# salemon/quattro-transformer-ilqr

Measured on AMD Instinct MI355X. Metric: iLQR iterations/sec (batch x horizon steps/s), quadrotor N=50 batch=4096, higher is better.
Workload: dtype f32; 1 GPU; quadrotor n_x=12 n_u=4 N=50, pure iLQR iteration = simulate (nominal rollout + cost) + linearisation and Riccati sweep (one fused launch) + 6-alpha line search/commit (BASELINE configs[2]; configs[3] when n_gpus=8); batch_per_gpu=4096, global_batch=4096, horizon=50, n_x=12, n_u=4, integrator=euler, parallelism=dp1 (independent trajectory shards)

## Files before the change

### quattro-transformer-ilqr_amd/csrc/quattro_device.h

```cpp
#pragma once
#include <hip/hip_runtime.h>

#include "../../include/quattro_hip.h"

#define QT_WAVE 64

#define QT_HD __host__ __device__ __forceinline__

template <int NX, int NU>
struct RowMajorRec {
  static constexpr int NZ = NX + NU;
  static constexpr int A = 0;
  static constexpr int B = A + NX * NX;
  static constexpr int LXX = B + NX * NU;
  static constexpr int LUX = LXX + NX * NX;
  static constexpr int LUU = LUX + NU * NX;
  static constexpr int LX = LUU + NU * NU;
  static constexpr int LU = LX + NX;
  static constexpr int SIZE = LU + NU;
  static constexpr int STRIDE = (SIZE + 3) / 4 * 4;
  static QT_HD int a(int i, int j) { return A + i * NX + j; }
  static QT_HD int b(int i, int a_) { return B + i * NU + a_; }
  static QT_HD int lxx(int i, int j) { return LXX + i * NX + j; }
  static QT_HD int lux(int a_, int j) { return LUX + a_ * NX + j; }
  static QT_HD int luu(int a_, int b_) { return LUU + a_ * NU + b_; }
  static QT_HD int lx(int i) { return LX + i; }
  static QT_HD int lu(int a_) { return LU + a_; }
};

struct Tile16Rec {
  static constexpr int NX = 12, NU = 4;
  static constexpr int F = 0, LXB = 192, LUU = 384, LZ = 400, SIZE = 416, STRIDE = 416;
  static QT_HD int zcol(int z) { return z < 12 ? (z / 3) * 4 + z % 3 : 4 * (z - 12) + 3; }
  static QT_HD int f(int i, int z) { return F + 3 * (16 * (i / 3) + zcol(z)) + i % 3; }
  static QT_HD int a(int i, int j) { return f(i, j); }
  static QT_HD int b(int i, int a_) { return f(i, 12 + a_); }
  static QT_HD int lxx(int i, int j) { return LXB + 4 * (12 * (i / 3) + j) + i % 3; }
  static QT_HD int lux(int a_, int j) { return LXB + 4 * (12 * a_ + j) + 3; }
  static QT_HD int luu(int a_, int b_) { return LUU + 4 * a_ + b_; }
  static QT_HD int lx(int i) { return LZ + i; }
  static QT_HD int lu(int a_) { return LZ + 12 + a_; }
};

struct Tile16CRec {
  static constexpr int NX = 12, NU = 4;
  static constexpr int F = 0, NDYN = 14, DUMP = 43, LUU = 44, LZ = 60, SIZE = 76, STRIDE = 76;
  static constexpr int HEADER = Tile16Rec::STRIDE;
  static QT_HD int dyn_index(int lane) {
    switch (lane) {
      case 19: return 0;  case 23: return 1;  case 24: return 2;  case 25: return 3;  case 26: return 4;
      case 27: return 5;  case 31: return 6;  case 40: return 7;  case 41: return 8;  case 45: return 9;
      case 46: return 10; case 60: return 11; case 61: return 12; case 62: return 13;
      default: return -1;
    }
// ... 51 lines not shown
struct PlantSpec {
  int integrator;
  float phys[8];
};

struct RefRows {
  const float* rows;
  int R, s, preview;
};
__device__ __forceinline__ int qt_ref_row(const RefRows& rr, int t) {
  const int i = rr.s + rr.preview * t;
  return i < rr.R - 1 ? i : rr.R - 1;
}
struct NoRef {
  __device__ __forceinline__ void operator()(int) const {}
};

namespace {
struct AlphaList {
  float a[QUATTRO_MAX_ALPHAS];
};
inline AlphaList make_alpha_list(const float* alphas, int n_alpha) {
  AlphaList al;
  for (int i = 0; i < QUATTRO_MAX_ALPHAS; ++i) al.a[i] = i < n_alpha ? alphas[i] : 0.0f;
  return al;
}
}

#define QT_DISPATCH_INTEG(p, ...)                                 \
  if ((p).integrator == QUATTRO_INTEGRATOR_EULER) {               \
    constexpr bool RK4 = false;                                   \
    __VA_ARGS__;                                                  \
  } else if ((p).integrator == QUATTRO_INTEGRATOR_RK4) {          \
    constexpr bool RK4 = true;                                    \
    __VA_ARGS__;                                                  \
  } else {                                                        \
    return QUATTRO_ERR_UNSUPPORTED;                               \
  }

__device__ __forceinline__ float qt_readlane(float v, int lane) {
  return __int_as_float(__builtin_amdgcn_readlane(__float_as_int(v), lane));
}

__device__ __forceinline__ float qt_sum_rows(float v) {
  int vi = __float_as_int(v);
  auto s16 = __builtin_amdgcn_permlane16_swap(vi, vi, false, false);
  float a = __int_as_float(s16[0]) + __int_as_float(s16[1]);
  int ai = __float_as_int(a);
  auto s32 = __builtin_amdgcn_permlane32_swap(ai, ai, false, false);
  return __int_as_float(s32[0]) + __int_as_float(s32[1]);
}

__device__ __forceinline__ bool qt_finite(float v) { return fabsf(v) <= 3.0e38f; }
```

### quattro-transformer-ilqr_amd/csrc/rollout_quad.hip

```cpp
#include "rollout_quad_body.h"

namespace {

template <bool RK4>
__global__ __launch_bounds__(64) void simulate_quad_kernel(const quattro_model_params p, const float* __restrict__ x0,
                                                           const float* __restrict__ u, int B, int N,
                                                           float* __restrict__ x, double* __restrict__ cost) {
  const int gid = blockIdx.x * blockDim.x + threadIdx.x;
  simulate_quad_body<RK4>(p, x0, u, N, x, cost, gid, (gid >> 2) < B);
}

template <bool RK4>
__global__ __launch_bounds__(64) void rollout_quad_kernel(const quattro_model_params p, const float* __restrict__ x_nom,
                                                          const float* __restrict__ u_nom, const float* __restrict__ K,
                                                          const float* __restrict__ k, AlphaList al, int n_alpha, int B,
                                                          int N, float* __restrict__ x_new, float* __restrict__ u_new,
                                                          double* __restrict__ cost, const int32_t* __restrict__ active) {
  const int gid = blockIdx.x * blockDim.x + threadIdx.x;
  const int b = gid >> 5, ai = (gid >> 2) & 7;
  const bool live = (b < B) && (active == nullptr || active[b < B ? b : 0] != 0);
  if (!__any(live)) return;
  const bool mine = live && ai < n_alpha;
  const size_t bb = live ? b : 0;
  const int aa = mine ? ai : 0;
  const LaneConst L = lane_const(p, gid & 3);
  const float* xn = x_nom + bb * (N + 1) * NX;
  const float* un = u_nom + bb * N * NU;
  const int wb = __builtin_amdgcn_readfirstlane(b);
  const NomSrc nom(L, x_nom, u_nom, K, k, N, wb, live ? b - wb : 0, 2);
  float alpha = al.a[0];
#pragma unroll
  for (int i = 1; i < QUATTRO_MAX_ALPHAS; ++i) alpha = (aa == i) ? al.a[i] : alpha;
  double J;
  if (x_new != nullptr && u_new != nullptr) {
    float* xo = x_new + ((size_t)aa * B + bb) * (N + 1) * NX;
    float* uo = u_new + ((size_t)aa * B + bb) * N * NU;
    if (mine && L.j < 3) {
#pragma unroll
      for (int g = 0; g < 4; ++g) xo[3 * g + L.a] = xn[3 * g + L.a];
    }
    J = quad_rollout_closed<RK4, 4, true, RK4>(p, L, nom, alpha, N, mine, ArrayStore(L, xo, uo, mine));
  } else {
    J = quad_rollout_closed<RK4, 4, true, RK4>(p, L, nom, alpha, N, mine, NoStore{});
  }
  J = quad_sum(J);
  if (mine && L.j == 0) cost[(size_t)ai * B + b] = J;
}

template <bool RK4>
__global__ __launch_bounds__(64) void linesearch_quad_kernel(const quattro_model_params p, float* x_nom, float* u_nom,
                                                             const float* __restrict__ K, const float* __restrict__ k,
                                                             AlphaList al, int n_alpha, int B, int N, double tol,
                                                             double* cost, int32_t* __restrict__ alpha_idx,
                                                             int32_t* active, int32_t* iters,
                                                             float* __restrict__ scratch) {
  linesearch_quad_body<RK4, 4, true, false, false, RK4>(p, x_nom, u_nom, K, k, al, n_alpha, B, N, tol, cost, alpha_idx, active, iters, scratch,
                                     blockIdx.x * blockDim.x + threadIdx.x, false);
}

__global__ __launch_bounds__(64) void track_quad_kernel(const float dt, const PlantSpec plant, const float* __restrict__ plant_phys,
                                                        const float* __restrict__ x0, const float* __restrict__ x_nom,
                                                        const float* __restrict__ u_nom, const float* __restrict__ K,
                                                        const int feedback, const int B, const int N, const int n_steps,
                                                        const float* __restrict__ disturbance, float* __restrict__ x_out,
                                                        float* __restrict__ u_out) {
  const int gid = blockIdx.x * blockDim.x + threadIdx.x;
  const int b = gid >> 2;
  const bool live = b < B;
  const size_t bb = live ? b : 0;
  const LaneConst L = lane_const_plant(plant, plant_phys, bb, dt, gid & 3);
  const int wb = __builtin_amdgcn_readfirstlane(b);
  const NomSrc nom(L, x_nom, u_nom, K, u_nom, N, wb, live ? b - wb : 0, 16);
  float xh[4];
#pragma unroll
  for (int g = 0; g < 4; ++g) xh[g] = x0[bb * NX + 3 * g + L.a];
  float* xrows = x_out + bb * (size_t)(n_steps + 1) * NX + L.a;
  if (live && L.j < 3) {
#pragma unroll
    for (int g = 0; g < 4; ++g) xrows[3 * g] = xh[g];
  }
  quad_track_body(L, plant.integrator == QUATTRO_INTEGRATOR_RK4, feedback != 0, nom, xh, n_steps,
                  disturbance != nullptr ? disturbance + bb * NX + L.a : nullptr, (size_t)B * NX, live, xrows,
                  u_out + bb * (size_t)n_steps * NU + L.j);
}

}

int quattro_launch_track_quad(const quattro_model_params& p, const PlantSpec& plant, const float* plant_phys, const float* x0,
                              const float* x_nom, const float* u_nom, const float* K, int feedback, int B, int N, int n_steps,
                              const float* disturbance, float* x_out, float* u_out, hipStream_t stream) {
  const long long tot = (long long)B * 4;
  hipLaunchKernelGGL(track_quad_kernel, dim3((unsigned)((tot + 63) / 64)), dim3(64), 0, stream, p.dt, plant, plant_phys, x0, x_nom,
                     u_nom, K, feedback, B, N, n_steps, disturbance, x_out, u_out);
  return hipGetLastError() == hipSuccess ? QUATTRO_OK : QUATTRO_ERR_LAUNCH;
}

int quattro_launch_simulate_quad(const quattro_model_params& p, const float* x0, const float* u, int B, int N, float* x,
                                 double* cost, hipStream_t stream) {
  const long long tot = (long long)B * 4;
  QT_DISPATCH_INTEG(p, hipLaunchKernelGGL((simulate_quad_kernel<RK4>), dim3((unsigned)((tot + 63) / 64)), dim3(64), 0,
                                         stream, p, x0, u, B, N, x, cost));
  return hipGetLastError() == hipSuccess ? QUATTRO_OK : QUATTRO_ERR_LAUNCH;
}

int quattro_launch_rollout_quad(const quattro_model_params& p, const float* x_nom, const float* u_nom, const float* K,
                                const float* k, const float* alphas, int n_alpha, int B, int N, float* x_new,
                                float* u_new, double* cost, const int32_t* active, hipStream_t stream) {
  const AlphaList al = make_alpha_list(alphas, n_alpha);
  const long long tot = (long long)B * 32;
// ... 17 lines not shown
```

### quattro-transformer-ilqr_amd/csrc/rollout_quad_body.h

```cpp
#pragma once
#include <type_traits>

#include "models_device.h"

namespace {

constexpr int NX = 12, NU = 4, CS = 16;

#define QT_QP(a, b, c, d) ((a) | ((b) << 2) | ((c) << 4) | ((d) << 6))
template <int CTRL>
__device__ __forceinline__ float quad_perm(float v) {
  return __builtin_bit_cast(float, __builtin_amdgcn_update_dpp(0, __builtin_bit_cast(int, v), CTRL, 0xf, 0xf, true));
}
template <int I>
__device__ __forceinline__ float quad_bcast(float v) {
  return quad_perm<QT_QP(I, I, I, I)>(v);
}
__device__ __forceinline__ double quad_sum(double v) {
  v += __shfl_xor(v, 1);
  v += __shfl_xor(v, 2);
  return v;
}

struct LaneConst {
// ... 390 lines not shown
}

template <bool RK4, int PF, bool PRIO, bool SHORTCUT, class Store, class RefS = NoRefSrc>
__device__ __forceinline__ double quad_rollout_closed(const quattro_model_params& p, const LaneConst& L,
                                                      const NomSrc& src, float alpha, int N, bool counted, Store store,
                                                      const RefS& ref = RefS()) {
  const unsigned long long counted_mask = barrier_lanes(p, counted);
  NomLane nb[PF];
#pragma unroll
  for (int d = 0; d < PF; ++d) nb[d].load(src, d < N ? d : N - 1);
  RefLane rl[PF], rlN;
#pragma unroll
  for (int d = 0; d < PF; ++d) rl[d].load(ref, d < N ? d : N - 1);
  rlN.load(ref, N);
  float xh[4];
#pragma unroll
  for (int g = 0; g < 4; ++g) xh[g] = nb[0].x[g];
  double J = 0.0;
  auto step = [&](const NomLane& b, const RefLane& rt, int t) __attribute__((always_inline)) {
    if constexpr (PRIO) __builtin_amdgcn_s_setprio(1);
    float dx[4];
#pragma unroll
    for (int g = 0; g < 4; ++g) dx[g] = xh[g] - b.x[g];
    const float du = gain_dot(b.K, dx, b.k);
    const float uh = fmaf(alpha, du, b.u);
    if constexpr (!PRIO) J += (double)lane_stage_cost<SHORTCUT>(p, with_ref<RefS>(L, rt), xh, uh, counted_mask);
    float xnext[4];
    const QuadU U(uh, Store::ALL_U);
    quad_step<RK4>(L, xh, U, xnext);
    if constexpr (PRIO) {
      __builtin_amdgcn_s_setprio(0);
      J += (double)lane_stage_cost<SHORTCUT>(p, with_ref<RefS>(L, rt), xh, uh, counted_mask);
    }
    store(L, t, U, xnext);
#pragma unroll
    for (int g = 0; g < 4; ++g) xh[g] = xnext[g];
  };
  int t = 0;
  for (; t + PF <= N; t += PF) {
#pragma unroll
    for (int d = 0; d < PF; ++d) {
      step(nb[d], rl[d], t + d);
      nb[d].load(src, t + d + PF < N ? t + d + PF : N - 1);
      rl[d].load(ref, t + d + PF < N ? t + d + PF : N - 1);
    }
  }
#pragma unroll
  for (int d = 0; d < PF - 1; ++d)
    if (t + d < N) step(nb[d], rl[d], t + d);
  J += (double)lane_final_cost(with_ref<RefS>(L, rlN), xh);
  return J;
}

template <bool RK4, bool PHYS = false, bool REF = false>
__device__ __forceinline__ void simulate_quad_body(const quattro_model_params& p, const float* __restrict__ x0,
                                                   const float* __restrict__ u, int N, float* __restrict__ x,
                                                   double* __restrict__ cost, const int gid, const bool live,
                                                   const float* __restrict__ model_phys = nullptr, const RefRows& rr = RefRows{}) {
  using RefS = std::conditional_t<REF, RefSrc, NoRefSrc>;
  const int b = gid >> 2;
  const size_t bb = live ? b : 0;
  const LaneConst L = lane_const_of<PHYS>(p, model_phys, bb, gid & 3);
  float* xo = x + bb * (N + 1) * NX + L.a;
  float xh[4];
#pragma unroll
  for (int g = 0; g < 4; ++g) xh[g] = x0[bb * NX + 3 * g + L.a];
  const bool writer = live && L.j < 3;
  const int bw = __builtin_amdgcn_readfirstlane(b);
  const __amdgpu_buffer_rsrc_t rsx =
      __builtin_amdgcn_make_buffer_rsrc(x + (size_t)bw * (N + 1) * NX, 0, 16 * (N + 1) * NX * 4, 0x00020000);
  const int vox = writer ? 4 * ((b - bw) * (N + 1) * NX + L.a) : 0x40000000;
  int uflags = 0x00020000;
  asm("" : "+s"(uflags));
  const __amdgpu_buffer_rsrc_t rsu =
      __builtin_amdgcn_make_buffer_rsrc(const_cast<float*>(u) + (size_t)bw * N * NU, 0, 16 * N * NU * 4, uflags);
  const int vou = 4 * ((live ? b - bw : 0) * N * NU + L.j);
  const int ou_last = (N - 1) * (NU * 4);
  auto control = [&](int ofs) __attribute__((always_inline)) {
    return __int_as_float(__builtin_amdgcn_raw_buffer_load_b32(rsu, vou, ofs < ou_last ? ofs : ou_last, 0));
  };
  if (writer) {
#pragma unroll
    for (int g = 0; g < 4; ++g) xo[3 * g] = xh[g];
  }
  const RefS ref(L, rr, bw, live ? b - bw : 0, 16);
  RefLane r0, r1, rN;
  r0.load(ref, 0);
  r1.load(ref, N > 1 ? 1 : 0);
  rN.load(ref, N);
  double J = 0.0;
  const unsigned long long live_mask = barrier_lanes(p, live);
  float u0 = control(0), u1 = control(NU * 4);
  int ou = 2 * (NU * 4);
  auto step = [&](float ut, const RefLane& rt, int t) __attribute__((always_inline)) {
    J += (double)lane_stage_cost(p, with_ref<RefS>(L, rt), xh, ut, live_mask);
    float xn[4];
    const QuadU U(ut);
    quad_step<RK4>(L, xh, U, xn);
#pragma unroll
    for (int g = 0; g < 4; ++g)
      __builtin_amdgcn_raw_buffer_store_b32(__float_as_int(xn[g]), rsx, vox + 12 * g, (t + 1) * (NX * 4), 0);
#pragma unroll
    for (int g = 0; g < 4; ++g) xh[g] = xn[g];
  };
  asm volatile("" : "+v"(u0), "+v"(u1));
  if constexpr (REF) {
#pragma unroll
    for (int g = 0; g < 4; ++g) asm volatile("" : "+v"(r0.xr[g]), "+v"(r1.xr[g]), "+v"(rN.xr[g]));
  }
  __builtin_amdgcn_s_waitcnt(0x0f70);
  int t = 0;
  for (; t + 1 < N; t += 2) {
    step(u0, r0, t);
    u0 = control(ou);
    ou += NU * 4;
    r0.load(ref, t + 2 < N ? t + 2 : N - 1);
    step(u1, r1, t + 1);
    u1 = control(ou);
    ou += NU * 4;
    r1.load(ref, t + 3 < N ? t + 3 : N - 1);
  }
  if (t < N) step(u0, r0, t);
  J += (double)lane_final_cost(with_ref<RefS>(L, rN), xh);
  J = quad_sum(J);
  if (live && L.j == 0 && cost != nullptr) cost[b] = J;
}

template <bool RK4, int PF, bool PRIO, bool PHYS = false, bool REF = false, bool SHORTCUT = true>
__device__ __forceinline__ void linesearch_quad_body(const quattro_model_params& p, float* x_nom, float* u_nom,
                                                     const float* __restrict__ K, const float* __restrict__ k,
                                                     const AlphaList& al, int n_alpha, int B, int N, double tol,
                                                     double* cost, int32_t* __restrict__ alpha_idx, int32_t* active,
                                                     int32_t* iters, float* __restrict__ scratch, const int gid,
                                                     const bool force, const float* __restrict__ model_phys = nullptr,
                                                     const RefRows& rr = RefRows{}) {
  const int b = gid >> 5, ai = (gid >> 2) & 7, l32 = gid & 31;
  const bool live = (b < B) && (force || active == nullptr || active[b < B ? b : 0] != 0);
  if (!__any(live)) return;
  const bool mine = live && ai < n_alpha;
  const size_t bb = live ? b : 0;
  const int aa = mine ? ai : 0;
  const LaneConst L = lane_const_of<PHYS>(p, model_phys, bb, gid & 3);
  float* xn = x_nom + bb * (N + 1) * NX;
  float* un = u_nom + bb * N * NU;
  const int wb = __builtin_amdgcn_readfirstlane(b);
  const NomSrc nom(L, x_nom, u_nom, K, k, N, wb, live ? b - wb : 0, 2);
  float* sc = scratch + (bb * 8) * (size_t)N * CS;
  float alpha = al.a[0];
#pragma unroll
  for (int i = 1; i < QUATTRO_MAX_ALPHAS; ++i) alpha = (aa == i) ? al.a[i] : alpha;
  const double J0 = live ? cost[bb] : 0.0;
  using RefS = std::conditional_t<REF, RefSrc, NoRefSrc>;
  double J = quad_rollout_closed<RK4, PF, PRIO, SHORTCUT>(p, L, nom, alpha, N, mine, ScratchStore(L, sc + (size_t)aa * N * CS, mine),
                                                RefS(L, rr, wb, live ? b - wb : 0, 2));
  J = quad_sum(J);
  const bool ok = mine && (J <= J0);
  const unsigned long long bal = __ballot(ok);
  const int lane = threadIdx.x & 63;
  const unsigned grp = (unsigned)((bal >> (lane & 32)) & 0x11111111ull);
  const int first = grp ? ((__ffs((int)grp) - 1) >> 2) : -1;
  if (live && first >= 0) {
    __builtin_amdgcn_fence(__ATOMIC_RELEASE, "workgroup");
    asm volatile("s_waitcnt vmcnt(0)" ::: "memory");
    __builtin_amdgcn_fence(__ATOMIC_ACQUIRE, "workgroup");
    const float* src = sc + (size_t)first * N * CS;
    const int e = l32 & 15, half = l32 >> 4;
    const bool isx = e < 12;
    const int slot = isx ? 4 * (e % 3) + e / 3 : e;
    float* dst = isx ? xn + NX + e : un + (e - 12);
    const int dstride = isx ? NX : NU;
    constexpr int COPY_U = 25;
    for (int t0 = half; t0 < N; t0 += 2 * COPY_U) {
      float v[COPY_U];
#pragma unroll
      for (int q = 0; q < COPY_U; ++q) {
        const int t = t0 + 2 * q;
        v[q] = src[(size_t)(t < N ? t : t0) * CS + slot];
      }
#pragma unroll
      for (int q = 0; q < COPY_U; ++q) {
        const int t = t0 + 2 * q;
        if (t < N) dst[(size_t)t * dstride] = v[q];
      }
    }
    if (ai == first && L.j == 0) {
      cost[b] = J;
      if (active != nullptr && fabs(J0 - J) < tol) active[b] = 0;
    }
  }
  if (live && l32 == 0) {
    if (alpha_idx != nullptr) alpha_idx[b] = first;
    if (iters != nullptr) iters[b] += 1;
    if (first < 0 && active != nullptr) active[b] = 0;
  }
}

}
```

### quattro-transformer-ilqr_amd/csrc/sweep_tile16.hip

```cpp
#include "sweep_tile16_body.h"

namespace {

constexpr int ROTATE_ABOVE_B = 256 * 4;

template <int MODE, bool ROTATE = false>
__global__ __launch_bounds__(QT_WAVE * WPB, 4) void sweep_tile16_kernel(const float* __restrict__ rec,
                                                               const float* __restrict__ VxN,
                                                               const float* __restrict__ VxxN, int S, float reg,
                                                               float* __restrict__ Kout, float* __restrict__ kout,
                                                               int32_t* __restrict__ status,
                                                               const int32_t* __restrict__ active,
                                                               const FusedArgs fa) {
  const int wv = __builtin_amdgcn_readfirstlane(threadIdx.x >> 6);
  const int b = blockIdx.x * WPB + wv;
  const int lane = threadIdx.x & 63;
  if (b >= fa.B) return;
  if (active != nullptr && active[b] == 0) return;
  __shared__ __attribute__((aligned(16))) float s_t_all[WPB * 16 * LD];
  __shared__ __attribute__((aligned(16))) float s_vx_all[WPB * 64];
  constexpr int LIN_FLOATS = sweep_lin_floats<MODE>();
  __shared__ __attribute__((aligned(16))) float s_lin_all[WPB * LIN_FLOATS];
  sweep_tile16_body<MODE, false, false, ROTATE>(rec, VxN, VxxN, S, reg, Kout, kout, status, fa, b, lane, s_t_all + wv * 16 * LD, s_vx_all + wv * 64,
                                                s_lin_all + wv * LIN_FLOATS);
}

}

int quattro_launch_sweep_tile16(const float* rec, const float* VxN, const float* VxxN, int B, int S, float reg,
                                float* K, float* k, int32_t* status, const int32_t* active, int layout, int n, int m,
                                hipStream_t stream) {
  FusedArgs none{};
  none.B = B;
  none.k_rows = 0;
  none.rn = n;
  none.rm = m;
  if (layout == QUATTRO_LAYOUT_ROWMAJOR_TILE) {
    if (n < 1 || n > 12 || m < 1 || m > 4) return QUATTRO_ERR_UNSUPPORTED;
    hipLaunchKernelGGL(sweep_tile16_kernel<MODE_ROWPAD>, dim3((B + WPB - 1) / WPB), dim3(QT_WAVE * WPB), 0, stream, rec, VxN, VxxN, S, reg, K, k,
                       status, active, none);
  } else if (layout == QUATTRO_LAYOUT_TILE16C)
    hipLaunchKernelGGL(sweep_tile16_kernel<MODE_COMPACT>, dim3((B + WPB - 1) / WPB), dim3(QT_WAVE * WPB), 0, stream, rec, VxN, VxxN, S, reg, K, k,
                       status, active, none);
  else if (layout == QUATTRO_LAYOUT_TILE16R)
    hipLaunchKernelGGL(sweep_tile16_kernel<MODE_DENSEF>, dim3((B + WPB - 1) / WPB), dim3(QT_WAVE * WPB), 0, stream, rec, VxN, VxxN, S, reg, K, k,
                       status, active, none);
  else
    hipLaunchKernelGGL(sweep_tile16_kernel<MODE_TILE16>, dim3((B + WPB - 1) / WPB), dim3(QT_WAVE * WPB), 0, stream, rec, VxN, VxxN, S, reg, K, k,
                       status, active, none);
  return hipGetLastError() == hipSuccess ? QUATTRO_OK : QUATTRO_ERR_LAUNCH;
}

int quattro_launch_sweep_fused(const quattro_model_params& p, const float* x, const float* u, int B, int N, int t_start,
                               float reg, float* K, float* k, int k_rows, int32_t* status, const int32_t* active,
                               hipStream_t stream) {
  const FusedArgs fa = fused_args(p, x, u, B, N, t_start, nullptr, k_rows);
  if (B > ROTATE_ABOVE_B)
    hipLaunchKernelGGL((sweep_tile16_kernel<MODE_FUSED, true>), dim3((B + WPB - 1) / WPB), dim3(QT_WAVE * WPB), 0, stream, nullptr, nullptr,
                       nullptr, N - t_start, reg, K, k, status, active, fa);
  else
    hipLaunchKernelGGL(sweep_tile16_kernel<MODE_FUSED>, dim3((B + WPB - 1) / WPB), dim3(QT_WAVE * WPB), 0, stream, nullptr, nullptr, nullptr,
                       N - t_start, reg, K, k, status, active, fa);
  return hipGetLastError() == hipSuccess ? QUATTRO_OK : QUATTRO_ERR_LAUNCH;
}

size_t quattro_sweep_fused_rk4_scratch_floats(int B, int S) { return (size_t)B * S * Rk4Coef::STRIDE; }
int quattro_launch_sweep_fused_rk4(const quattro_model_params& p, const float* x, const float* u, int B, int N, int t_start,
                                   float reg, float* K, float* k, int k_rows, int32_t* status, const int32_t* active,
                                   float* coef, hipStream_t stream) {
  const FusedArgs fa = fused_args(p, x, u, B, N, t_start, coef, k_rows);
  hipLaunchKernelGGL(sweep_tile16_kernel<MODE_FUSED_RK4>, dim3((B + WPB - 1) / WPB), dim3(QT_WAVE * WPB), 0, stream, nullptr, nullptr,
                     nullptr, N - t_start, reg, K, k, status, active, fa);
  return hipGetLastError() == hipSuccess ? QUATTRO_OK : QUATTRO_ERR_LAUNCH;
}
```

### quattro-transformer-ilqr_amd/csrc/sweep_tile16_body.h

```cpp
#pragma once
#include "models_device.h"

namespace {

typedef float f32x4 __attribute__((ext_vector_type(4)));

struct StepRegs {
  float f0, f1, f2;
  f32x4 lq;
  float lz;
};

struct LanePtrs {
  const float* pf;
  const float* plq;
  const float* plz;
  bool dynf, dynq;
};

template <int STRIDE, bool HDR>
__device__ __forceinline__ StepRegs load_step(const LanePtrs& lp, int s) {
  StepRegs o;
  const int off = s * STRIDE;
  const int offf = (!HDR || lp.dynf) ? off : 0, offq = (!HDR || lp.dynq) ? off : 0;
// ... 163 lines not shown
  for (int a = 0; a < 4; ++a) {
    float lu = 2.0f * p.r[a] * us[a], luu = 2.0f * p.r[a];
    if (p.barrier_alpha != 0.0f && !skip) {
      const float sp = qt_softplus(-us[a], p.barrier_beta), sg = qt_sigmoid(-p.barrier_beta * us[a]);
      lu = fmaf(p.barrier_alpha, -2.0f * sp * sg, lu);
      luu = fmaf(p.barrier_alpha, 2.0f * sg * sg + 2.0f * sp * p.barrier_beta * sg * (1.0f - sg), luu);
    }
    lz[NX + a] = lu;
    luud[a] = luu;
  }
#pragma unroll
  for (int q = 0; q < 4; ++q) emit(Rk4Coef::LZ / 4 + q, make_float4(lz[4 * q], lz[4 * q + 1], lz[4 * q + 2], lz[4 * q + 3]));
  emit(Rk4Coef::LUUD / 4, make_float4(luud[0], luud[1], luud[2], luud[3]));
}

template <class Emit>
__device__ __forceinline__ void rk4_step_coefs(const quattro_model_params& p, const float* ph, const float* xs, const float* us,
                                               Emit emit) {
  rk4_step_coefs(p, ph, p.x_ref, xs, us, emit);
}

struct Rk4Entry {
  int idx;
  float cst;
};
__device__ __forceinline__ Rk4Entry rk4_m_entry(const float* ph, int row_tile, int col_tile) {
  Rk4Entry e{Rk4Tab::ZERO, 0.0f};
  if ((row_tile & 3) == 3) return e;
  const int i = 3 * (row_tile >> 2) + (row_tile & 3);
  const bool uc = (col_tile & 3) == 3;
  const int g = col_tile >> 2, j = 3 * g + (col_tile & 3);
  if (uc) {
    if (i == 3) e.idx = 3;
    else if (i == 4) e.idx = 7;
    else if (i == 5) e.idx = 10;
    else if (i == 9) e.cst = ((g == 1 || g == 2) ? 1.0f : -1.0f) * (ph[4] / ph[1]);
    else if (i == 10) e.cst = (g < 2 ? 1.0f : -1.0f) * (ph[4] / ph[2]);
    else if (i == 11) e.cst = ((g & 1) ? -1.0f : 1.0f) * (ph[6] / ph[3]);
    return e;
  }
  if (i < 3) { if (j == i + 3) e.cst = 1.0f; return e; }
  if (i == 3) { if (j == 6) e.idx = 0; else if (j == 7) e.idx = 1; else if (j == 8) e.idx = 2; return e; }
  if (i == 4) { if (j == 6) e.idx = 4; else if (j == 7) e.idx = 5; else if (j == 8) e.idx = 6; return e; }
  if (i == 5) { if (j == 6) e.idx = 8; else if (j == 7) e.idx = 9; return e; }
  if (i == 6) { if (j == 6) e.idx = 11; else if (j == 7) e.idx = 12; else if (j == 9) e.cst = 1.0f; else if (j == 10) e.idx = 13; else if (j == 11) e.idx = 14; return e; }
  if (i == 7) { if (j == 6) e.idx = 15; else if (j == 10) e.idx = 16; else if (j == 11) e.idx = 17; return e; }
  if (i == 8) { if (j == 6) e.idx = 18; else if (j == 7) e.idx = 19; else if (j == 10) e.idx = 20; else if (j == 11) e.idx = 21; return e; }
  if (i == 9) { if (j == 10) e.idx = 22; else if (j == 11) e.idx = 23; return e; }
  if (i == 10) { if (j == 9) e.idx = 24; else if (j == 11) e.idx = 25; return e; }
  if (j == 9) e.idx = 26; else if (j == 10) e.idx = 27;
  return e;
}

template <int MODE, bool PHYS = false, bool REF = false, bool ROTATE = false>
__device__ __forceinline__ bool sweep_tile16_body(const float* __restrict__ rec, const float* __restrict__ VxN,
                                                  const float* __restrict__ VxxN, int S, float reg,
                                                  float* __restrict__ Kout, float* __restrict__ kout,
                                                  int32_t* __restrict__ status, const FusedArgs& fa, const int b,
                                                  const int lane, float* s_t, float* s_vx, float* s_lin,
                                                  const float* model_phys = nullptr, const RefRows& rr = RefRows{}) {
  static_assert(!ROTATE || MODE == MODE_FUSED, "the favourite changes at the refills of the fused Euler mode");
  static_assert(!(PHYS || REF) || MODE == MODE_FUSED || MODE == MODE_FUSED_RK4, "per-trajectory parameters: the fused modes only");
  const float* rows_b = nullptr;
  if constexpr (REF) rows_b = rr.rows + (size_t)__builtin_amdgcn_readfirstlane(b) * rr.R * 12;
  float phv[8];
  if constexpr (PHYS) {
    typedef const float __attribute__((address_space(4))) * ConstRow;
    const ConstRow row = (ConstRow)model_phys + 8 * (size_t)__builtin_amdgcn_readfirstlane(b);
#pragma unroll
    for (int i = 0; i < 8; ++i) phv[i] = row[i];
  }
  const float* const ph = PHYS ? phv : fa.p.phys;
  QuadQuot qq{};
  if constexpr (MODE == MODE_FUSED) qq = PHYS ? quad_quot(fa.p.dt, ph) : fa.quot;
  constexpr bool ROWPAD = MODE == MODE_ROWPAD;
  constexpr bool COMPACT = MODE != MODE_TILE16 && !ROWPAD;
  constexpr int REC_STRIDE = MODE == MODE_TILE16 ? Tile16Rec::STRIDE : MODE == MODE_DENSEF ? Tile16RRec::STRIDE : Tile16CRec::STRIDE;
  constexpr bool FUSED = MODE == MODE_FUSED;
  constexpr bool RK4F = MODE == MODE_FUSED_RK4;
  constexpr bool CHECK_PIVOTS = MODE == MODE_TILE16 || ROWPAD;
  const int pn = ROWPAD ? fa.rn : 12, pm = ROWPAD ? fa.rm : 4;
  const int r = lane >> 4, c = lane & 15, g = c >> 2, sp = c & 3;
  const bool ucol = (sp == 3);
  const int xj = 3 * g + (ucol ? 0 : sp);
  const float regadd = (c == 4 * r + 3) ? reg : 0.0f;
  const int c4 = 4 * c, a16 = 4 * (lane ^ 16), a32 = 4 * (lane ^ 32);

  float vA0 = 0.0f, vA1 = 0.0f, vA2 = 0.0f;
  float vx0, vx1, vx2;
  if constexpr (FUSED || RK4F) {
    const float* xN = fa.x + ((size_t)b * (fa.N + 1) + fa.N) * 12;
    if (!ucol) {
      vA0 = (xj == 3 * r + 0) ? 2.0f * fa.p.qf[xj] : 0.0f;
      vA1 = (xj == 3 * r + 1) ? 2.0f * fa.p.qf[xj] : 0.0f;
      vA2 = (xj == 3 * r + 2) ? 2.0f * fa.p.qf[xj] : 0.0f;
    }
    const float* const xrN = REF ? rows_b + 12 * qt_ref_row(rr, fa.N) : fa.p.x_ref;
    vx0 = 2.0f * fa.p.qf[3 * r + 0] * (xN[3 * r + 0] - xrN[3 * r + 0]);
    vx1 = 2.0f * fa.p.qf[3 * r + 1] * (xN[3 * r + 1] - xrN[3 * r + 1]);
    vx2 = 2.0f * fa.p.qf[3 * r + 2] * (xN[3 * r + 2] - xrN[3 * r + 2]);
    if constexpr (FUSED) {
      static_assert(sweep_lin_floats<MODE>() % 4 == 0, "the LDS slice is zeroed in 16-byte pieces");
      for (int i = lane; i < sweep_lin_floats<MODE>() / 4; i += QT_WAVE) reinterpret_cast<f32x4*>(s_lin)[i] = f32x4{0.0f, 0.0f, 0.0f, 0.0f};
      wave_sync();
      if (lane == 0) EulerRecord<QUATTRO_MODEL_QUADROTOR, Tile16Rec>::fill_const(s_lin, fa.p, qq);
      if (lane < FUSED_BATCH)
        EulerRecord<QUATTRO_MODEL_QUADROTOR, Tile16FRec>::fill_const(s_lin + Tile16Rec::STRIDE + lane * Tile16FRec::STRIDE, fa.p, qq);
      wave_sync();
    }
  } else if constexpr (ROWPAD) {
    const float* pv = VxxN + (size_t)b * pn * pn;
    const float* pg = VxN + (size_t)b * pn;
    const bool cj = !ucol && xj < pn;
    const int i0 = 3 * r, xjc = cj ? xj : 0;
    vA0 = (cj && i0 + 0 < pn) ? pv[xjc * pn + (i0 + 0 < pn ? i0 + 0 : 0)] : 0.0f;
    vA1 = (cj && i0 + 1 < pn) ? pv[xjc * pn + (i0 + 1 < pn ? i0 + 1 : 0)] : 0.0f;
    vA2 = (cj && i0 + 2 < pn) ? pv[xjc * pn + (i0 + 2 < pn ? i0 + 2 : 0)] : 0.0f;
    vx0 = i0 + 0 < pn ? pg[i0 + 0] : 0.0f;
    vx1 = i0 + 1 < pn ? pg[i0 + 1 < pn ? i0 + 1 : 0] : 0.0f;
    vx2 = i0 + 2 < pn ? pg[i0 + 2 < pn ? i0 + 2 : 0] : 0.0f;
  } else {
    if (!ucol) {
      const float* pv = VxxN + (size_t)b * 144 + xj * 12 + 3 * r;
      vA0 = pv[0];
      vA1 = pv[1];
      vA2 = pv[2];
    }
    vx0 = VxN[(size_t)b * 12 + 3 * r + 0];
    vx1 = VxN[(size_t)b * 12 + 3 * r + 1];
    vx2 = VxN[(size_t)b * 12 + 3 * r + 2];
  }

  if (ucol) {
    vA0 = vx0;
    vA1 = vx1;
    vA2 = vx2;
  }

  LanePtrs lp;
  int pad_of[8] = {0, 0, 0, 0, 0, 0, 0, 0}, pad_stride = 0;
  const float* pad_base = nullptr;
  constexpr int FZQ = Tile16FRec::LZ + 12 - Tile16FRec::LUUD, RZQ = Rk4Tab::LUUD - 12;
  static_assert(FZQ > 0 && FZQ <= Tile16FRec::LZ && RZQ >= 0 && 16 + RZQ <= Rk4Tab::COST_STEP, "l_uu and l_z from one base, inside the record");
  int of_z = 0;
  unsigned af = 0, af_step = 0, aq = 0;
  f32x4 lqc = {0.0f, 0.0f, 0.0f, 0.0f};
  const bool qsel = ucol && (g == r);
  if constexpr (RK4F) {
    lp.dynf = true;
    lp.dynq = ucol;
    lp.pf = lp.plq = lp.plz = nullptr;
    of_z = Rk4Tab::COST + (ucol ? 12 + g : xj);
    if (!ucol) {
// ... 223 lines not shown
    b2 = load(cnt > 2 ? cnt - 3 : 0);
    int s = cnt - 1;
    for (; s >= 2; s -= 3) {
      step(prio, b0, base + s);
      b0 = load(s >= 3 ? s - 3 : 0);
      step(prio, b1, base + s - 1);
      b1 = load(s >= 4 ? s - 4 : 0);
      step(prio, b2, base + s - 2);
      b2 = load(s >= 5 ? s - 5 : 0);
    }
    if (s >= 0) step(prio, b0, base + s);
    if (s >= 1) step(prio, b1, base + s - 1);
  };
  if constexpr (RK4F) {
    float* coef = fa.coef + (size_t)b * S * Rk4Coef::STRIDE;
    for (int c0 = 0; c0 < S; c0 += QT_WAVE) {
      const int ls = c0 + lane;
      if (ls < S) {
        const int t = fa.t_start + ls;
        const float4* px = reinterpret_cast<const float4*>(fa.x + ((size_t)b * (fa.N + 1) + t) * 12);
        const float4 xa = px[0], xb = px[1], xc = px[2];
        const float4 ua = *reinterpret_cast<const float4*>(fa.u + ((size_t)b * fa.N + t) * 4);
        const float xs[12] = {xa.x, xa.y, xa.z, xa.w, xb.x, xb.y, xb.z, xb.w, xc.x, xc.y, xc.z, xc.w};
        const float us[4] = {ua.x, ua.y, ua.z, ua.w};
        float4* dst = reinterpret_cast<float4*>(coef) + ls;
        const float* const xr = REF ? rows_b + 12 * qt_ref_row(rr, t) : fa.p.x_ref;
        rk4_step_coefs(fa.p, ph, xr, xs, us, [&](int q, float4 v) __attribute__((always_inline)) { dst[(size_t)q * S] = v; });
      }
    }
    __builtin_amdgcn_fence(__ATOMIC_RELEASE, "workgroup");
    asm volatile("s_waitcnt vmcnt(0)" ::: "memory");
    __builtin_amdgcn_fence(__ATOMIC_ACQUIRE, "workgroup");
    const float4* coef4 = reinterpret_cast<const float4*>(coef);
    for (int i = lane; i < Rk4Tab::FLOATS; i += QT_WAVE) s_lin[i] = 0.0f;
    const int top = ((S - 1) / RK4_BATCH) * RK4_BATCH;
    for (int base = top; base >= 0; base -= RK4_BATCH) {
      const int cnt = S - base < RK4_BATCH ? S - base : RK4_BATCH;
      wave_sync();
      for (int e = lane; e < cnt * Rk4Coef::PIECES; e += QT_WAVE) {
        const int sl = e / Rk4Coef::PIECES, q = e - sl * Rk4Coef::PIECES;
        const float4 v = coef4[(size_t)q * S + base + sl];
        float* dst = q < 28 ? s_lin + sl * Rk4Tab::STEP + (q / 7) * Rk4Tab::STAGE + 4 * (q % 7)
                            : s_lin + Rk4Tab::COST + sl * Rk4Tab::COST_STEP + 4 * (q - 28);
        *reinterpret_cast<float4*>(dst) = v;
      }
      wave_sync();
      run(StepPrio<2, 1, 0>{}, cnt, base);
    }
  } else if constexpr (FUSED) {
    float* stage = s_lin + Tile16Rec::STRIDE;
    const int sl = lane & 31;
    const bool dynl = (lane < 32) == (sl < 13);
    const int ca = dynl ? 0 : 2;
    const float ra0 = dynl ? fa.p.r[0] : fa.p.r[2], ra1 = dynl ? fa.p.r[1] : fa.p.r[3];
    float4 xa, xb, xc, ua;
    float4 ra, rb, rc;
    auto fetch = [&](int base) __attribute__((always_inline)) {
      const int cnt = S - base < FUSED_BATCH ? S - base : FUSED_BATCH;
      const int t = fa.t_start + base + (sl < cnt ? sl : 0);
      const float4* px = reinterpret_cast<const float4*>(fa.x + ((size_t)b * (fa.N + 1) + t) * 12);
      xa = px[0];
      xb = px[1];
      xc = px[2];
      ua = *reinterpret_cast<const float4*>(fa.u + ((size_t)b * fa.N + t) * 4);
      if constexpr (REF) {
        const float4* pr = reinterpret_cast<const float4*>(rows_b + 12 * qt_ref_row(rr, t));
        ra = pr[0];
        rb = pr[1];
        rc = pr[2];
      }
    };
    const int top = ((S - 1) / FUSED_BATCH) * FUSED_BATCH;
    fetch(top);
    for (int base = top; base >= 0; base -= FUSED_BATCH) {
      const int cnt = S - base < FUSED_BATCH ? S - base : FUSED_BATCH;
      wave_sync();
      {
        using ER = EulerRecord<QUATTRO_MODEL_QUADROTOR, Tile16FRec>;
        const float xs[12] = {xa.x, xa.y, xa.z, xa.w, xb.x, xb.y, xb.z, xb.w, xc.x, xc.y, xc.z, xc.w};
        const float us[4] = {ua.x, ua.y, ua.z, ua.w};
        float xrv[12];
        if constexpr (REF) {
          const float v[12] = {ra.x, ra.y, ra.z, ra.w, rb.x, rb.y, rb.z, rb.w, rc.x, rc.y, rc.z, rc.w};
#pragma unroll
          for (int i = 0; i < 12; ++i) xrv[i] = v[i];
        }
        const float* const xr = REF ? xrv : fa.p.x_ref;
        constexpr bool SHORT_CUTS = ROTATE;
        QuadTrig tr;
        if constexpr (SHORT_CUTS) {
          qt_sincos_chain(dynl ? xs[6] : xs[8], &tr.sph, &tr.cph);
          qt_sincos_chain(xs[7], &tr.sth, &tr.cth);
        } else {
          qt_sincos(dynl ? xs[6] : xs[8], &tr.sph, &tr.cph);
          qt_sincos(xs[7], &tr.sth, &tr.cth);
        }
        tr.sps = __int_as_float(__builtin_amdgcn_ds_bpermute(a32, __float_as_int(tr.sph)));
        tr.cps = __int_as_float(__builtin_amdgcn_ds_bpermute(a32, __float_as_int(tr.cph)));
        const float uc0 = dynl ? us[0] : us[2], uc1 = dynl ? us[1] : us[3];
        bool skip = false;
        if constexpr (SHORT_CUTS)
          skip = qt_all_lanes(qt_barrier_derivs_negligible(fa.p, ra0, uc0) & qt_barrier_derivs_negligible(fa.p, ra1, uc1));
        if (sl < cnt) {
          float* mine = stage + sl * Tile16FRec::STRIDE;
          if (dynl) {
            quad_trig_finish(tr);
            ER::fill_dynamics(mine, fa.p, ph[0], qq, tr, xs, us);
          } else {
            ER::fill_lx(mine, fa.p, xr, xs);
          }
          ER::fill_control(mine, fa.p, ca, ra0, uc0, skip);
          ER::fill_control(mine, fa.p, ca + 1, ra1, uc1, skip);
        }
      }
      if (base > 0) fetch(base - FUSED_BATCH);
      wave_sync();
      if constexpr (ROTATE) {
        const bool favourite = ((batches + slot) & 3) == 3;
        ++batches;
        if (favourite) run(StepPrio<3, 3, 2>{}, cnt, base);
        else run(StepPrio<2, 1, 0>{}, cnt, base);
      } else {
        run(StepPrio<2, 1, 0>{}, cnt, base);
      }
    }
  } else {
// ... 14 lines not shown
```

Before: 2.051 billion steps/s.

## Issue kernel-entry loads early and deepen simulate ring in quad kernels

Adds a kernarg-segment prefetch helper that touches every cache line of each kernel's argument block at entry. It also hoists the first global loads (the active flag, nominal cost, lane constants, the first fused-sweep batch and terminal state) ahead of the early-exit checks. The simulate rollout grows its control/reference prefetch ring from 2 to 4 steps and stores the initial state after the waitcnt. The aim is to hide launch-time scalar and global load latency in these short kernels. In exchange, trajectories that exit early still issue loads, and the deeper ring raises register pressure.

```diff
diff --git a/quattro-transformer-ilqr_amd/csrc/quattro_device.h b/quattro-transformer-ilqr_amd/csrc/quattro_device.h
--- a/quattro-transformer-ilqr_amd/csrc/quattro_device.h
+++ b/quattro-transformer-ilqr_amd/csrc/quattro_device.h
@@ -1,5 +1,7 @@
 #pragma once
 #include <hip/hip_runtime.h>
+
+#include <type_traits>
 
 #include "../../include/quattro_hip.h"
 
@@ -157,3 +159,49 @@
 }
 
 __device__ __forceinline__ bool qt_finite(float v) { return fabsf(v) <= 3.0e38f; }
+
+template <int I, int N, class F>
+__device__ __forceinline__ void qt_static_for_from(F& f) {
+  if constexpr (I < N) {
+    f(std::integral_constant<int, I>{});
+    qt_static_for_from<I + 1, N>(f);
+  }
+}
+template <int N, class F>
+__device__ __forceinline__ void qt_static_for(F f) {
+  qt_static_for_from<0, N>(f);
+}
+
+template <class... Args>
+constexpr int qt_kernarg_bytes() {
+  int off = 0;
+  const int size[] = {(int)sizeof(Args)...}, align[] = {(int)alignof(Args)...};
+  for (int i = 0; i < (int)sizeof...(Args); ++i) off = (off + align[i] - 1) / align[i] * align[i] + size[i];
+  return off;
+}
+template <int LINES>
+__device__ __forceinline__ void qt_kernarg_touch(const uint32_t __attribute__((address_space(4))) * ka, int last) {
+  static_assert(LINES <= 12, "one operand of the asm statement per load");
+  uint32_t v[12];
+#pragma unroll
+  for (int i = 0; i < 12; ++i) v[i] = ka[i + 1 < LINES ? 16 * i : last];
+  asm volatile("" ::"s"(v[0]), "s"(v[1]), "s"(v[2]), "s"(v[3]), "s"(v[4]), "s"(v[5]), "s"(v[6]), "s"(v[7]), "s"(v[8]), "s"(v[9]),
+               "s"(v[10]), "s"(v[11]));
+}
+template <class... Args>
+__device__ __forceinline__ void qt_kernarg_prefetch() {
+  constexpr int BYTES = qt_kernarg_bytes<Args...>();
+  static_assert(BYTES >= 4 && BYTES % 4 == 0, "a segment of whole dwords");
+  typedef const uint32_t __attribute__((address_space(4))) * KernArg;
+  qt_kernarg_touch<(BYTES + 63) / 64 + 1>((KernArg)__builtin_amdgcn_kernarg_segment_ptr(), BYTES / 4 - 1);
+}
+template <class Kernel>
+struct QtKernArgs;
+template <class... Args>
+struct QtKernArgs<void (*)(Args...)> {
+  static __device__ __forceinline__ void prefetch() { qt_kernarg_prefetch<Args...>(); }
+};
+template <class Kernel>
+__device__ __forceinline__ void qt_kernarg_prefetch_of() {
+  QtKernArgs<Kernel>::prefetch();
+}
diff --git a/quattro-transformer-ilqr_amd/csrc/rollout_quad.hip b/quattro-transformer-ilqr_amd/csrc/rollout_quad.hip
--- a/quattro-transformer-ilqr_amd/csrc/rollout_quad.hip
+++ b/quattro-transformer-ilqr_amd/csrc/rollout_quad.hip
@@ -6,8 +6,9 @@
 __global__ __launch_bounds__(64) void simulate_quad_kernel(const quattro_model_params p, const float* __restrict__ x0,
                                                            const float* __restrict__ u, int B, int N,
                                                            float* __restrict__ x, double* __restrict__ cost) {
+  qt_kernarg_prefetch_of<decltype(&simulate_quad_kernel<RK4>)>();
   const int gid = blockIdx.x * blockDim.x + threadIdx.x;
-  simulate_quad_body<RK4>(p, x0, u, N, x, cost, gid, (gid >> 2) < B);
+  simulate_quad_body<RK4, false, false, SIM_RING, true>(p, x0, u, N, x, cost, gid, (gid >> 2) < B);
 }
 
 template <bool RK4>
@@ -54,7 +55,8 @@
                                                              double* cost, int32_t* __restrict__ alpha_idx,
                                                              int32_t* active, int32_t* iters,
                                                              float* __restrict__ scratch) {
-  linesearch_quad_body<RK4, 4, true, false, false, RK4>(p, x_nom, u_nom, K, k, al, n_alpha, B, N, tol, cost, alpha_idx, active, iters, scratch,
+  qt_kernarg_prefetch_of<decltype(&linesearch_quad_kernel<RK4>)>();
+  linesearch_quad_body<RK4, 4, true, false, false, RK4, true>(p, x_nom, u_nom, K, k, al, n_alpha, B, N, tol, cost, alpha_idx, active, iters, scratch,
                                      blockIdx.x * blockDim.x + threadIdx.x, false);
 }
 
diff --git a/quattro-transformer-ilqr_amd/csrc/rollout_quad_body.h b/quattro-transformer-ilqr_amd/csrc/rollout_quad_body.h
--- a/quattro-transformer-ilqr_amd/csrc/rollout_quad_body.h
+++ b/quattro-transformer-ilqr_amd/csrc/rollout_quad_body.h
@@ -466,7 +466,8 @@
   return J;
 }
 
-template <bool RK4, bool PHYS = false, bool REF = false>
+constexpr int SIM_RING = 4;
+template <bool RK4, bool PHYS = false, bool REF = false, int RING = 2, bool ENTRY = false>
 __device__ __forceinline__ void simulate_quad_body(const quattro_model_params& p, const float* __restrict__ x0,
                                                    const float* __restrict__ u, int N, float* __restrict__ x,
                                                    double* __restrict__ cost, const int gid, const bool live,
@@ -493,19 +494,21 @@
   auto control = [&](int ofs) __attribute__((always_inline)) {
     return __int_as_float(__builtin_amdgcn_raw_buffer_load_b32(rsu, vou, ofs < ou_last ? ofs : ou_last, 0));
   };
-  if (writer) {
-#pragma unroll
-    for (int g = 0; g < 4; ++g) xo[3 * g] = xh[g];
+  if constexpr (!ENTRY) {
+    if (writer) {
+#pragma unroll
+      for (int g = 0; g < 4; ++g) xo[3 * g] = xh[g];
+    }
   }
   const RefS ref(L, rr, bw, live ? b - bw : 0, 16);
-  RefLane r0, r1, rN;
-  r0.load(ref, 0);
-  r1.load(ref, N > 1 ? 1 : 0);
+  RefLane rq[RING], rN;
+  qt_static_for<RING>([&](auto d) __attribute__((always_inline)) { rq[d].load(ref, d < N ? d : 0); });
   rN.load(ref, N);
   double J = 0.0;
   const unsigned long long live_mask = barrier_lanes(p, live);
-  float u0 = control(0), u1 = control(NU * 4);
-  int ou = 2 * (NU * 4);
+  float uq[RING];
+  qt_static_for<RING>([&](auto d) __attribute__((always_inline)) { uq[d] = control(d * (NU * 4)); });
+  int ou = RING * (NU * 4);
   auto step = [&](float ut, const RefLane& rt, int t) __attribute__((always_inline)) {
     J += (double)lane_stage_cost(p, with_ref<RefS>(L, rt), xh, ut, live_mask);
     float xn[4];
@@ -517,30 +520,50 @@
 #pragma unroll
     for (int g = 0; g < 4; ++g) xh[g] = xn[g];
   };
-  asm volatile("" : "+v"(u0), "+v"(u1));
+  if constexpr (ENTRY) {
+    asm volatile("" : "+v"(xh[0]), "+v"(xh[1]), "+v"(xh[2]), "+v"(xh[3]));
+#pragma unroll
+    for (int d = 0; d < RING; ++d) asm volatile("" : "+v"(uq[d]));
+  } else {
+    static_assert(ENTRY || RING == 2, "the persistent loops' form");
+    asm volatile("" : "+v"(uq[0]), "+v"(uq[1]));
+  }
   if constexpr (REF) {
-#pragma unroll
-    for (int g = 0; g < 4; ++g) asm volatile("" : "+v"(r0.xr[g]), "+v"(r1.xr[g]), "+v"(rN.xr[g]));
+    if constexpr (ENTRY) {
+#pragma unroll
+      for (int d = 0; d < RING; ++d)
+#pragma unroll
+        for (int g = 0; g < 4; ++g) asm volatile("" : "+v"(rq[d].xr[g]));
+#pragma unroll
+      for (int g = 0; g < 4; ++g) asm volatile("" : "+v"(rN.xr[g]));
+    } else {
+#pragma unroll
+      for (int g = 0; g < 4; ++g) asm volatile("" : "+v"(rq[0].xr[g]), "+v"(rq[1].xr[g]), "+v"(rN.xr[g]));
+    }
   }
   __builtin_amdgcn_s_waitcnt(0x0f70);
+  if constexpr (ENTRY) {
+#pragma unroll
+    for (int g = 0; g < 4; ++g) __builtin_amdgcn_raw_buffer_store_b32(__float_as_int(xh[g]), rsx, vox + 12 * g, 0, 0);
+  }
   int t = 0;
-  for (; t + 1 < N; t += 2) {
-    step(u0, r0, t);
-    u0 = control(ou);
-    ou += NU * 4;
-    r0.load(ref, t + 2 < N ? t + 2 : N - 1);
-    step(u1, r1, t + 1);
-    u1 = control(ou);
-    ou += NU * 4;
-    r1.load(ref, t + 3 < N ? t + 3 : N - 1);
-  }
-  if (t < N) step(u0, r0, t);
+  for (; t + (RING - 1) < N; t += RING) {
+    qt_static_for<RING>([&](auto d) __attribute__((always_inline)) {
+      step(uq[d], rq[d], t + d);
+      uq[d] = control(ou);
+      ou += NU * 4;
+      rq[d].load(ref, t + d + RING < N ? t + d + RING : N - 1);
+    });
+  }
+  qt_static_for<RING - 1>([&](auto d) __attribute__((always_inline)) {
+    if (t + d < N) step(uq[d], rq[d], t + d);
+  });
   J += (double)lane_final_cost(with_ref<RefS>(L, rN), xh);
   J = quad_sum(J);
   if (live && L.j == 0 && cost != nullptr) cost[b] = J;
 }
 
-template <bool RK4, int PF, bool PRIO, bool PHYS = false, bool REF = false, bool SHORTCUT = true>
+template <bool RK4, int PF, bool PRIO, bool PHYS = false, bool REF = false, bool SHORTCUT = true, bool ENTRY = false>
 __device__ __forceinline__ void linesearch_quad_body(const quattro_model_params& p, float* x_nom, float* u_nom,
                                                      const float* __restrict__ K, const float* __restrict__ k,
                                                      const AlphaList& al, int n_alpha, int B, int N, double tol,
@@ -549,12 +572,29 @@
                                                      const bool force, const float* __restrict__ model_phys = nullptr,
                                                      const RefRows& rr = RefRows{}) {
   const int b = gid >> 5, ai = (gid >> 2) & 7, l32 = gid & 31;
-  const bool live = (b < B) && (force || active == nullptr || active[b < B ? b : 0] != 0);
+  bool live;
+  double J0 = 0.0;
+  LaneConst L;
+  if constexpr (ENTRY) {
+    const int bc = b < B ? b : 0;
+    const int32_t* const fp = active != nullptr ? active + bc : reinterpret_cast<const int32_t*>(cost + bc);
+    const bool flag = (*fp != 0) | force | (active == nullptr);
+    J0 = cost[bc];
+    if constexpr (!PHYS) {
+      L = lane_const(p, gid & 3);
+      asm volatile("" : "+v"(L.rj));
+    }
+    asm volatile("" : "+v"(J0));
+    live = (b < B) && flag;
+  } else {
+    live = (b < B) && (force || active == nullptr || active[b < B ? b : 0] != 0);
+  }
   if (!__any(live)) return;
   const bool mine = live && ai < n_alpha;
   const size_t bb = live ? b : 0;
   const int aa = mine ? ai : 0;
-  const LaneConst L = lane_const_of<PHYS>(p, model_phys, bb, gid & 3);
+  if constexpr (!ENTRY || PHYS) L = lane_const_of<PHYS>(p, model_phys, bb, gid & 3);
+  if constexpr (ENTRY) J0 = live ? J0 : 0.0;
   float* xn = x_nom + bb * (N + 1) * NX;
   float* un = u_nom + bb * N * NU;
   const int wb = __builtin_amdgcn_readfirstlane(b);
@@ -563,7 +603,7 @@
   float alpha = al.a[0];
 #pragma unroll
   for (int i = 1; i < QUATTRO_MAX_ALPHAS; ++i) alpha = (aa == i) ? al.a[i] : alpha;
-  const double J0 = live ? cost[bb] : 0.0;
+  if constexpr (!ENTRY) J0 = live ? cost[bb] : 0.0;
   using RefS = std::conditional_t<REF, RefSrc, NoRefSrc>;
   double J = quad_rollout_closed<RK4, PF, PRIO, SHORTCUT>(p, L, nom, alpha, N, mine, ScratchStore(L, sc + (size_t)aa * N * CS, mine),
                                                 RefS(L, rr, wb, live ? b - wb : 0, 2));
diff --git a/quattro-transformer-ilqr_amd/csrc/sweep_tile16.hip b/quattro-transformer-ilqr_amd/csrc/sweep_tile16.hip
--- a/quattro-transformer-ilqr_amd/csrc/sweep_tile16.hip
+++ b/quattro-transformer-ilqr_amd/csrc/sweep_tile16.hip
@@ -12,17 +12,23 @@
                                                                int32_t* __restrict__ status,
                                                                const int32_t* __restrict__ active,
                                                                const FusedArgs fa) {
+  qt_kernarg_prefetch_of<decltype(&sweep_tile16_kernel<MODE, ROTATE>)>();
   const int wv = __builtin_amdgcn_readfirstlane(threadIdx.x >> 6);
   const int b = blockIdx.x * WPB + wv;
   const int lane = threadIdx.x & 63;
   if (b >= fa.B) return;
-  if (active != nullptr && active[b] == 0) return;
+  const int32_t* flag = nullptr;
+  if constexpr (MODE == MODE_FUSED) {
+    if (active != nullptr) flag = active + b;
+  } else {
+    if (active != nullptr && active[b] == 0) return;
+  }
   __shared__ __attribute__((aligned(16))) float s_t_all[WPB * 16 * LD];
   __shared__ __attribute__((aligned(16))) float s_vx_all[WPB * 64];
   constexpr int LIN_FLOATS = sweep_lin_floats<MODE>();
   __shared__ __attribute__((aligned(16))) float s_lin_all[WPB * LIN_FLOATS];
-  sweep_tile16_body<MODE, false, false, ROTATE>(rec, VxN, VxxN, S, reg, Kout, kout, status, fa, b, lane, s_t_all + wv * 16 * LD, s_vx_all + wv * 64,
-                                                s_lin_all + wv * LIN_FLOATS);
+  sweep_tile16_body<MODE, false, false, ROTATE, MODE == MODE_FUSED>(rec, VxN, VxxN, S, reg, Kout, kout, status, fa, b, lane, s_t_all + wv * 16 * LD, s_vx_all + wv * 64,
+                                                s_lin_all + wv * LIN_FLOATS, nullptr, RefRows{}, flag);
 }
 
 }
diff --git a/quattro-transformer-ilqr_amd/csrc/sweep_tile16_body.h b/quattro-transformer-ilqr_amd/csrc/sweep_tile16_body.h
--- a/quattro-transformer-ilqr_amd/csrc/sweep_tile16_body.h
+++ b/quattro-transformer-ilqr_amd/csrc/sweep_tile16_body.h
@@ -239,14 +239,17 @@
   return e;
 }
 
-template <int MODE, bool PHYS = false, bool REF = false, bool ROTATE = false>
+template <int MODE, bool PHYS = false, bool REF = false, bool ROTATE = false, bool ENTRY = false>
 __device__ __forceinline__ bool sweep_tile16_body(const float* __restrict__ rec, const float* __restrict__ VxN,
                                                   const float* __restrict__ VxxN, int S, float reg,
                                                   float* __restrict__ Kout, float* __restrict__ kout,
                                                   int32_t* __restrict__ status, const FusedArgs& fa, const int b,
                                                   const int lane, float* s_t, float* s_vx, float* s_lin,
-                                                  const float* model_phys = nullptr, const RefRows& rr = RefRows{}) {
+                                                  const float* model_phys = nullptr, const RefRows& rr = RefRows{},
+                                                  const int32_t* __restrict__ flag = nullptr) {
   static_assert(!ROTATE || MODE == MODE_FUSED, "the favourite changes at the refills of the fused Euler mode");
+  static_assert(!ENTRY || MODE == MODE_FUSED, "the early requests are the fused Euler mode's");
+  constexpr bool EARLY = ENTRY;
   static_assert(!(PHYS || REF) || MODE == MODE_FUSED || MODE == MODE_FUSED_RK4, "per-trajectory parameters: the fused modes only");
   const float* rows_b = nullptr;
   if constexpr (REF) rows_b = rr.rows + (size_t)__builtin_amdgcn_readfirstlane(b) * rr.R * 12;
@@ -275,17 +278,61 @@
 
   float vA0 = 0.0f, vA1 = 0.0f, vA2 = 0.0f;
   float vx0, vx1, vx2;
+  float4 xa, xb, xc, ua;
+  float4 ra, rb, rc;
+  auto fetch = [&](int base) __attribute__((always_inline)) {
+    const int cnt = S - base < FUSED_BATCH ? S - base : FUSED_BATCH;
+    const int t = fa.t_start + base + ((lane & 31) < cnt ? (lane & 31) : 0);
+    const float4* px = reinterpret_cast<const float4*>(fa.x + ((size_t)b * (fa.N + 1) + t) * 12);
+    xa = px[0];
+    xb = px[1];
+    xc = px[2];
+    ua = *reinterpret_cast<const float4*>(fa.u + ((size_t)b * fa.N + t) * 4);
+    if constexpr (REF) {
+      const float4* pr = reinterpret_cast<const float4*>(rows_b + 12 * qt_ref_row(rr, t));
+      ra = pr[0];
+      rb = pr[1];
+      rc = pr[2];
+    }
+  };
+  float ra0e = 0.0f, ra1e = 0.0f;
   if constexpr (FUSED || RK4F) {
+    if constexpr (EARLY) {
+      fetch(((S - 1) / FUSED_BATCH) * FUSED_BATCH);
+      const bool dl = (lane < 32) == ((lane & 31) < 13);
+      ra0e = dl ? fa.p.r[0] : fa.p.r[2];
+      ra1e = dl ? fa.p.r[1] : fa.p.r[3];
+    }
     const float* xN = fa.x + ((size_t)b * (fa.N + 1) + fa.N) * 12;
-    if (!ucol) {
-      vA0 = (xj == 3 * r + 0) ? 2.0f * fa.p.qf[xj] : 0.0f;
-      vA1 = (xj == 3 * r + 1) ? 2.0f * fa.p.qf[xj] : 0.0f;
-      vA2 = (xj == 3 * r + 2) ? 2.0f * fa.p.qf[xj] : 0.0f;
-    }
-    const float* const xrN = REF ? rows_b + 12 * qt_ref_row(rr, fa.N) : fa.p.x_ref;
-    vx0 = 2.0f * fa.p.qf[3 * r + 0] * (xN[3 * r + 0] - xrN[3 * r + 0]);
-    vx1 = 2.0f * fa.p.qf[3 * r + 1] * (xN[3 * r + 1] - xrN[3 * r + 1]);
-    vx2 = 2.0f * fa.p.qf[3 * r + 2] * (xN[3 * r + 2] - xrN[3 * r + 2]);
+    if constexpr (EARLY) {
+      const float* const xrN = REF ? rows_b + 12 * qt_ref_row(rr, fa.N) : fa.p.x_ref;
+      const float qfj = fa.p.qf[xj];
+      float tq[3], tx[3], tr[3];
+#pragma unroll
+      for (int q = 0; q < 3; ++q) {
+        tq[q] = fa.p.qf[3 * r + q];
+        tx[q] = xN[3 * r + q];
+        tr[q] = xrN[3 * r + q];
+      }
+      if (flag != nullptr && *flag == 0) return false;
+      const float qf2 = 2.0f * qfj;
+      vA0 = (!ucol && xj == 3 * r + 0) ? qf2 : 0.0f;
+      vA1 = (!ucol && xj == 3 * r + 1) ? qf2 : 0.0f;
+      vA2 = (!ucol && xj == 3 * r + 2) ? qf2 : 0.0f;
+      vx0 = 2.0f * tq[0] * (tx[0] - tr[0]);
+      vx1 = 2.0f * tq[1] * (tx[1] - tr[1]);
+      vx2 = 2.0f * tq[2] * (tx[2] - tr[2]);
+    } else {
+      if (!ucol) {
+        vA0 = (xj == 3 * r + 0) ? 2.0f * fa.p.qf[xj] : 0.0f;
+        vA1 = (xj == 3 * r + 1) ? 2.0f * fa.p.qf[xj] : 0.0f;
+        vA2 = (xj == 3 * r + 2) ? 2.0f * fa.p.qf[xj] : 0.0f;
+      }
+      const float* const xrN = REF ? rows_b + 12 * qt_ref_row(rr, fa.N) : fa.p.x_ref;
+      vx0 = 2.0f * fa.p.qf[3 * r + 0] * (xN[3 * r + 0] - xrN[3 * r + 0]);
+      vx1 = 2.0f * fa.p.qf[3 * r + 1] * (xN[3 * r + 1] - xrN[3 * r + 1]);
+      vx2 = 2.0f * fa.p.qf[3 * r + 2] * (xN[3 * r + 2] - xrN[3 * r + 2]);
+    }
     if constexpr (FUSED) {
       static_assert(sweep_lin_floats<MODE>() % 4 == 0, "the LDS slice is zeroed in 16-byte pieces");
       for (int i = lane; i < sweep_lin_floats<MODE>() / 4; i += QT_WAVE) reinterpret_cast<f32x4*>(s_lin)[i] = f32x4{0.0f, 0.0f, 0.0f, 0.0f};
@@ -615,26 +662,9 @@
     const int sl = lane & 31;
     const bool dynl = (lane < 32) == (sl < 13);
     const int ca = dynl ? 0 : 2;
-    const float ra0 = dynl ? fa.p.r[0] : fa.p.r[2], ra1 = dynl ? fa.p.r[1] : fa.p.r[3];
-    float4 xa, xb, xc, ua;
-    float4 ra, rb, rc;
-    auto fetch = [&](int base) __attribute__((always_inline)) {
-      const int cnt = S - base < FUSED_BATCH ? S - base : FUSED_BATCH;
-      const int t = fa.t_start + base + (sl < cnt ? sl : 0);
-      const float4* px = reinterpret_cast<const float4*>(fa.x + ((size_t)b * (fa.N + 1) + t) * 12);
-      xa = px[0];
-      xb = px[1];
-      xc = px[2];
-      ua = *reinterpret_cast<const float4*>(fa.u + ((size_t)b * fa.N + t) * 4);
-      if constexpr (REF) {
-        const float4* pr = reinterpret_cast<const float4*>(rows_b + 12 * qt_ref_row(rr, t));
-        ra = pr[0];
-        rb = pr[1];
-        rc = pr[2];
-      }
-    };
+    const float ra0 = EARLY ? ra0e : (dynl ? fa.p.r[0] : fa.p.r[2]), ra1 = EARLY ? ra1e : (dynl ? fa.p.r[1] : fa.p.r[3]);
     const int top = ((S - 1) / FUSED_BATCH) * FUSED_BATCH;
-    fetch(top);
+    if constexpr (!EARLY) fetch(top);
     for (int base = top; base >= 0; base -= FUSED_BATCH) {
       const int cnt = S - base < FUSED_BATCH ? S - base : FUSED_BATCH;
       wave_sync();
```

Result: faster. 2.080 billion steps/s, median of 6 (+1.4%).
